# JiaoXianjun/multi-rtl-sdr-calibration

Hardware: AMD Instinct MI355X
Metric: IQ Msamples/s through FCCH+SCH calib (higher is better)
Workload: dtype f64; 1 GPU; cfg4 full chain gsm_sync_demod.m:107-124: 64 dongle streams (64/GPU) x 1020000 IQ samples (102 frames), fir1(46), FCCH+SCH+total_ppm_calculation, table on the host; streams_per_gpu=64, streams_total=64, output=table, collective=none, rows_checked_vs_oracle_per_rank=0

## Files before the change

### multi-rtl-sdr-calibration_amd/csrc/kernels_detect.h

```cpp
#pragma once
#include "state.h"
#include "kernels_frontend.h"

__device__ __forceinline__ constexpr int fft16_rev(int k) { return ((k & 1) << 3) | ((k & 2) << 1) | ((k & 4) >> 1) | ((k & 8) >> 3); }
__device__ __forceinline__ void fft16(cplx* x) {
    const double c1 = 0.92387953251128673848, s1 = 0.38268343236508978178;
    const double r2 = 0.70710678118654752440;
    const cplx w16[8] = {{1.0, 0.0}, {c1, -s1}, {r2, -r2}, {s1, -c1}, {0.0, -1.0}, {-s1, -c1}, {-r2, -r2}, {-c1, -s1}};
#pragma unroll
    for (int len = 16; len >= 2; len >>= 1) {
        const int half = len >> 1, step = 16 / len;
#pragma unroll
        for (int i = 0; i < 16; i += len) {
#pragma unroll
            for (int j = 0; j < half; ++j) {
                const cplx u = x[i + j], v = x[i + j + half];
                x[i + j] = make_double2(u.x + v.x, u.y + v.y);
                const cplx d = make_double2(u.x - v.x, u.y - v.y);
                const int t = j * step;
                if (t == 0) x[i + j + half] = d;
                else if (t == 4) x[i + j + half] = make_double2(d.y, -d.x);
                else x[i + j + half] = cmul(d, w16[t]);
            }
        }
// ... 1257 lines not shown
        qr = fma(u.x - v.x, t.y, qr); qi = fma(u.y - v.y, t.y, qi);
    }
    *Xa = make_double2(pr - qi, pi + qr);
    *Xb = make_double2(pr + qi, pi - qr);
}

__global__ void k_make_twiddles(cplx* tw, int n) {
    const int i = blockIdx.x * blockDim.x + threadIdx.x;
    if (i >= n) return;
    double sn, cs;
    sincospi(-2.0 * (double)i / (double)n, &sn, &cs);
    tw[i] = make_double2(cs, sn);
}

#define FFT_THREADS 512
#define FC_NB 8
template <int MODE>
__global__ void __launch_bounds__(FFT_THREADS) k_fft_burst(const StreamState* __restrict__ sts,
                                                           const cplx* __restrict__ win, long win_stream_stride,
                                                           long win_stride, int nfft,
                                                           const cplx* __restrict__ tw_g, PeakOut* __restrict__ peaks,
                                                           cplx* __restrict__ x0, int H) {
    extern __shared__ __attribute__((aligned(16))) unsigned char smem[];
    const int N2 = nfft / 37;
    const int ldb = N2 + 1;
    cplx* xs = (cplx*)smem;
    cplx* B = xs + nfft;
    cplx* w37 = B + 37 * ldb;
    cplx* wN2 = w37 + 40;
    __shared__ double red_p[FFT_THREADS / 64];
    __shared__ int red_t[FFT_THREADS / 64], red_k[FFT_THREADS / 64];
// ... 25 lines not shown
        const int ok = __shfl_down(key, off, 64);
        const int okk = __shfl_down(kk, off, 64);
        if (op > best || (op == best && ok < key)) { best = op; key = ok; kk = okk; }
    }
    const int wv = tid >> 6;
    if ((tid & 63) == 0) { red_p[wv] = best; red_t[wv] = key; red_k[wv] = kk; }
    __syncthreads();
    if (tid == 0) {
        for (int i = 1; i < FFT_THREADS / 64; ++i)
            if (red_p[i] > best || (red_p[i] == best && red_t[i] < key)) { best = red_p[i]; key = red_t[i]; kk = red_k[i]; }
        PeakOut o; o.p = best; o.tie = key; o.k = kk;
        peaks[(size_t)s * H + w] = o;
    }
}

#define FS_CHUNK 64
#define FS_ERR_SCALE_CHUNK 0.0001220703125

template <int NB = 19>
__device__ __forceinline__ cplx anchor_dft(const cplx* xw, int k, const cplx* __restrict__ tw_g, int nfft, int lane) {
    double ar = 0.0, ai = 0.0;
    const int stp = (int)(((unsigned)k * 64u) % (unsigned)nfft);
    int idx = (int)(((unsigned)k * (unsigned)lane) % (unsigned)nfft);
    for (int n0 = 0; n0 < nfft; n0 += NB * 64) {
        cplx t[NB];
        int id = idx;
#pragma unroll
        for (int u = 0; u < NB; ++u) {
            t[u] = tw_g[id];
            id += stp;
            if (id >= nfft) id -= nfft;
// ... 309 lines not shown
        if (res) *res = o2; else peak_store(&out[(size_t)s * H + w], o2);
    }
}

__device__ __forceinline__ float fc_group8_sum(float v) {
    int t;
    t = __builtin_amdgcn_update_dpp(0, __float_as_int(v), 0xB1, 0xF, 0xF, true);
    v += __int_as_float(t);
    t = __builtin_amdgcn_update_dpp(0, __float_as_int(v), 0x4E, 0xF, 0xF, true);
    v += __int_as_float(t);
    t = __builtin_amdgcn_update_dpp(0, __float_as_int(v), 0x141, 0xF, 0xF, true);
    v += __int_as_float(t);
    return v;
}

__host__ __device__ constexpr int fc_gcd64(int n) { int b = 64; while (n % b) b >>= 1; return b; }
__host__ __device__ constexpr int fc_threads(int nshift) {
    return ((nshift - 1) / FS_CHUNK * FC_NB + 63) / 64 * 64 < 256 ? 256 : ((nshift - 1) / FS_CHUNK * FC_NB + 63) / 64 * 64;
}
#define FC_XP(p) ((p) + ((p) >> 7))
struct FusedGather {
    const uint8_t* raw; long raw_stride;
    const double* coef;
    cplx* win_out;
    int ntaps, per;
    int sym47, pad;
};
__host__ inline size_t fc_stage_bytes(int per, int ntaps) {
    const int span8 = per + ntaps + 8;
    return (size_t)(span8 + span8 / 4 + 1) * sizeof(cplx) + (size_t)fir_taps_padded(ntaps) * sizeof(double);
}

struct FcCarve {
    int nstep, wlen, B, nA, nM, nchunk, ld1;
    size_t xs, reg1, reg2;
    size_t Sp, Et, tw1, tw2, sumS, Cs, sh_scan, sh_scan2;
    size_t total, launch, stage;
};
__host__ __device__ constexpr FcCarve fc_carve(int nshift, int nfft) {
    FcCarve c{};
    c.nstep = nshift - 1; c.wlen = c.nstep + nfft;
    c.B = fc_gcd64(nfft); c.nA = nfft / c.B; c.nM = c.wlen / c.B; c.nchunk = c.nstep / FS_CHUNK;
    c.ld1 = c.B + 2;
    const int xp = FC_XP(c.nstep + 2);
    const size_t r1 = (size_t)FC_NB * c.nM * sizeof(cplx), e1 = (size_t)(c.nstep + 2) * sizeof(double);
    const size_t r2 = (size_t)FC_NB * (c.B + 2 + nfft / c.B) * sizeof(cplx), e2 = (size_t)2 * (size_t)(xp + 1) * sizeof(float) + 16 * sizeof(double);
    c.xs = 0;
    c.reg1 = (size_t)FC_XP(c.wlen) * sizeof(cplx);
    c.reg2 = c.reg1 + (r1 > e1 ? r1 : e1);
    c.Sp = c.Et = c.reg1;
    c.tw1 = c.reg2;
    c.tw2 = c.tw1 + (size_t)(FC_NB * c.ld1) * sizeof(cplx);
    c.sumS = c.reg2;
    c.Cs = c.sumS + (size_t)xp * sizeof(float);
    c.sh_scan = c.Cs + (size_t)(xp + (xp & 1)) * sizeof(float);
    c.sh_scan2 = c.sh_scan + 8 * sizeof(double);
    c.total = c.reg2 + (r2 > e2 ? r2 : e2);
    c.launch = (c.total + 15) & ~(size_t)15;
    c.stage = c.launch - c.reg1 - 16;
    return c;
}
static_assert(fc_carve(1025, 1184).total == 53520, "reference geometry: with the 144 bytes of static LDS, 100 bytes under the 53 760-byte line (three workgroups per CU)");
template <typename T>
__device__ __forceinline__ T* fc_at(size_t off) {
    extern __shared__ __attribute__((aligned(16))) unsigned char smem[];
    return (T*)(smem + off);
}
struct FcThread { int tid, lane, wave, nthr, nwave; };
struct alignas(16) FcShared { double red_p[8]; int red_t[8], red_k[8]; int a, b, lo; };

#define FC_PRIO(P0, P1, P2) if (gridDim.x * gridDim.y <= 768u) { const unsigned rnd_ = (blockIdx.y * gridDim.x + blockIdx.x) >> 8; if (rnd_ == 0) __builtin_amdgcn_s_setprio(P0); else if (rnd_ == 1) __builtin_amdgcn_s_setprio(P1); else __builtin_amdgcn_s_setprio(P2); }
#define FC_PF 8
#ifdef GSMCAL_DEVTIMING
#define FC_ROLE_STAMP(wv, i)                                                                                          \
    do {                                                                                                              \
        if (DEV_STAMP_ON(KID_CERT, i) && g_stamps && th.wave == (wv) && th.lane == 0 && blockIdx.y * gridDim.x + blockIdx.x < DEV_STAMP_BLOCKS) \
            g_stamps[((size_t)KID_CERT * DEV_STAMP_BLOCKS + blockIdx.y * gridDim.x + blockIdx.x) * 16 + (i)] = wall_clock64();           \
// ... 186 lines not shown
    for (int a = 0; a < nA; ++a) {
        const cplx v = sb[a], t = tb[a * FC_NB];
        xr = fma(v.x, t.x, fma(-v.y, t.y, xr));
        xi = fma(v.x, t.y, fma(v.y, t.x, xi));
    }
}

__device__ __forceinline__ double fc_energy_term(const cplx& a1, const cplx& b1) {
    return (a1.x * a1.x + a1.y * a1.y) - (b1.x * b1.x + b1.y * b1.y);
}
__device__ __forceinline__ double fc_slack_term(const cplx& a1, const cplx& b1) {
    const double dr = a1.x - b1.x, di = a1.y - b1.y;
    return (double)(__fsqrt_rn((float)(dr * dr + di * di)) * 1.00000095367431640625f);
}

template <int OV>
__device__ __forceinline__ void fc_scan_role(const FcCarve& cv, const FcThread& th, int nfft, bool we) {
    const int lane = th.lane, nstep = cv.nstep;
    cplx* xs = fc_at<cplx>(cv.xs);
    double* Et = fc_at<double>(cv.Et);
    float* Cs = fc_at<float>(cv.Cs);
    const int per = OV > 0 ? 2 * OV : (nstep + 63) >> 6;
    const int i0 = lane * per < nstep ? lane * per : nstep, i1 = i0 + per < nstep ? i0 + per : nstep;
    auto term = [&](int q) -> double {
        const cplx a1 = xs[FC_XP(q + nfft)], b1 = xs[FC_XP(q)];
        if (we) return fc_energy_term(a1, b1);
        return fc_slack_term(a1, b1);
    };
    double run = 0.0;
    if (we) {
        for (int i = lane; i < nfft; i += 64) { const cplx v = xs[FC_XP(i)]; run += v.x * v.x + v.y * v.y; }
        for (int off = 32; off > 0; off >>= 1) run += __shfl_down(run, off, 64);
        run = __shfl(run, 0, 64);
    }
    double g[OV > 0 ? 2 * OV : 1];
    double loc = 0.0;
    if (OV > 0) {
#pragma unroll
        for (int u = 0; u < 2 * OV; ++u) { g[u] = term(i0 + u); loc += g[u]; }
    } else {
        for (int q = i0; q < i1; ++q) loc += term(q);
    }
    double inc = loc;
    for (int off = 1; off < 64; off <<= 1) {
        const double o = __shfl_up(inc, off, 64);
        if (lane >= off) inc += o;
    }
    const double exc = __shfl_up(inc, 1, 64);
    if (lane > 0) run += exc;
    if (OV > 0) {
#pragma unroll
        for (int u = 0; u < 2 * OV; ++u) {
            if (we) Et[i0 + u] = run; else Cs[FC_XP(i0 + u)] = (float)run;
            run += g[u];
        }
    } else {
        for (int q = i0; q < i1; ++q) {
            if (we) Et[q] = run; else Cs[FC_XP(q)] = (float)run;
            run += term(q);
        }
    }
    if (i1 == nstep && i0 < nstep) { if (we) Et[nstep] = run; else Cs[FC_XP(nstep)] = (float)run; }
}

__device__ __forceinline__ void fc_scan_block(const FcCarve& cv, const FcThread& th, int nfft, FcShared& sh) {
    const int tid = th.tid, lane = th.lane, wave = th.wave, nthr = th.nthr, nwave = th.nwave, nstep = cv.nstep;
    cplx* xs = fc_at<cplx>(cv.xs);
    double* Et = fc_at<double>(cv.Et);
    float* Cs = fc_at<float>(cv.Cs);
    double* sh_scan = fc_at<double>(cv.sh_scan);
    double* sh_scan2 = fc_at<double>(cv.sh_scan2);
    double e0 = 0.0;
    for (int i = tid; i < nfft; i += nthr) { const cplx v = xs[FC_XP(i)]; e0 += v.x * v.x + v.y * v.y; }
    for (int off = 32; off > 0; off >>= 1) e0 += __shfl_down(e0, off, 64);
    if (lane == 0) sh.red_p[wave] = e0;
    const int per = (nstep + nthr - 1) / nthr;
    const int i0 = tid * per < nstep ? tid * per : nstep, i1 = i0 + per < nstep ? i0 + per : nstep;
// ... 29 lines not shown
        const int ot = __shfl_down(bt, off, 64);
        const int ok = __shfl_down(bk, off, 64);
        if (op > best || (op == best && (ot < bt || (ot == bt && ok < bk)))) { best = op; bt = ot; bk = ok; }
    }
}
__device__ __forceinline__ void fc_block_best(const FcThread& th, FcShared& sh, double& best, int& bt, int& bk) {
    if (th.lane == 0) { sh.red_p[th.wave] = best; sh.red_t[th.wave] = bt; sh.red_k[th.wave] = bk; }
    __syncthreads();
    best = sh.red_p[0]; bt = sh.red_t[0]; bk = sh.red_k[0];
    for (int i = 1; i < th.nwave; ++i)
        if (sh.red_p[i] > best || (sh.red_p[i] == best && (sh.red_t[i] < bt || (sh.red_t[i] == bt && sh.red_k[i] < bk)))) {
            best = sh.red_p[i]; bt = sh.red_t[i]; bk = sh.red_k[i];
        }
}

__device__ __forceinline__ void fc_certificate(const FcCarve& cv, const FcThread& th, int nfft, FcShared& sh, double best, int bt) {
    const int tid = th.tid, lane = th.lane, wave = th.wave, nthr = th.nthr, nwave = th.nwave, nstep = cv.nstep;
    double* Et = fc_at<double>(cv.Et);
    float* sumS = fc_at<float>(cv.sumS);
    float* Cs = fc_at<float>(cv.Cs);
    double* sh_scan = fc_at<double>(cv.sh_scan);
    double* sh_scan2 = fc_at<double>(cv.sh_scan2);
    const double INF = __longlong_as_double(0x7ff0000000000000LL);
    const double sb = best > 0.0 ? sqrt(best) * (1.0 - 1e-9) : -1.0;
    const int per = (nstep + nthr) / nthr;
    const int u0 = tid * per < nstep + 1 ? tid * per : nstep + 1, u1 = u0 + per < nstep + 1 ? u0 + per : nstep + 1;
    double mf = INF, mb = INF;
    for (int t = u0; t < u1; ++t) {
        const double NE = (double)nfft * Et[t];
        const float ss = sumS[FC_XP(t)];
        const double R = NE - (double)ss + 4e-6 * NE;
        float sf = ss <= 3.0e38f ? __fsqrt_rn((float)(R > 0.0 ? R : 0.0)) * 1.000001f : __int_as_float(0x7f800000);
        if (!(sf >= 0.0f)) sf = __int_as_float(0x7f800000);
        sumS[FC_XP(t)] = sf;
        const double ct = (double)Cs[FC_XP(t)];
        mf = fmin(mf, (double)sf - ct);
        mb = fmin(mb, (double)sf + ct);
    }
    double pf = mf, pb = mb;
    for (int off = 1; off < 64; off <<= 1) {
        const double o = __shfl_up(pf, off, 64), ob = __shfl_down(pb, off, 64);
        if (lane >= off) pf = fmin(pf, o);
        if (lane + off < 64) pb = fmin(pb, ob);
    }
// ... 62 lines not shown
    FC_PRIO(0, 1, 2)
    if (fg.raw) {
        fc_window_raw<OV, NTAPS>(cv, th, fg, sts + s, (const unsigned short*)(fg.raw + (size_t)s * fg.raw_stride), sts[s].win_start[w],
                                 fg.win_out + (size_t)s * win_stream_stride + (size_t)w * win_stride);
        if (th.tid == 0) { sh.a = 0; sh.b = cv.nstep; }
        __syncthreads();
    } else {
        fc_window_load(cv, th, win + (size_t)s * win_stream_stride + (size_t)w * win_stride);
        if (th.tid == 0) { sh.a = 0; sh.b = cv.nstep; }
        __syncthreads();
    }
    DEV_STAMP(KID_CERT, blockIdx.y * gridDim.x + blockIdx.x, 1);
    FC_PRIO(2, 1, 0)
    const int lo = fc_choose_bins(cv, th, nfft, tw_g, sh);
    DEV_STAMP(KID_CERT, blockIdx.y * gridDim.x + blockIdx.x, 2);
    const int j = th.tid & (FC_NB - 1), c = th.tid / FC_NB;
    const bool act = c < cv.nchunk;
    const int k = ((lo + j) % nfft + nfft) % nfft;
    fc_twiddles(cv, th, nfft, lo, tw_g);
    __syncthreads();
    fc_level1(cv, th, j, c);
    __syncthreads();
    DEV_STAMP(KID_CERT, blockIdx.y * gridDim.x + blockIdx.x, 3);
    double xr = 0.0, xi = 0.0;
    if (act) fc_level2_anchor(cv, j, c, xr, xi);
    __syncthreads();
    DEV_STAMP(KID_CERT, blockIdx.y * gridDim.x + blockIdx.x, 4);
    FC_PRIO(0, 1, 2)
    const int nslide = (FC_NB * cv.nchunk + 63) >> 6;
    const bool split = th.nwave - nslide >= 2;
    if (split) {
        DEV_STAMP(KID_CERT, blockIdx.y * gridDim.x + blockIdx.x, 5);
        if (th.wave == nslide || th.wave == nslide + 1) {
            const bool we = th.wave == nslide;
            fc_scan_role<OV>(cv, th, nfft, we);
            FC_ROLE_STAMP(th.wave, we ? 12 : 13);
        }
    } else {
        fc_scan_block(cv, th, nfft, sh);
        DEV_STAMP(KID_CERT, blockIdx.y * gridDim.x + blockIdx.x, 5);
    }
    double best = -1.0;
    int bt = 0x7fffffff;
    if (act) {
        cplx* xs = fc_at<cplx>(cv.xs);
        float* sumS = fc_at<float>(cv.sumS);
        const cplx wk = tw_g[k];
        const double wr = wk.x, wi = -wk.y;
        const int t0 = c * FS_CHUNK;
        if (c == 0) {
            const double p = xr * xr + xi * xi;
// ... 17 lines not shown
                xi = ar * wi + ai * wr;
                const double p = xr * xr + xi * xi;
                if (p > best) { best = p; bt = t0 + q0 + u + 1; }
                ps[u] = fc_group8_sum((float)p);
            }
#pragma unroll
            for (int u = 0; u < FC_PF; ++u) sumS[FC_XP(t0 + q0 + u + 1)] = ps[u];
        }
    }
    FC_ROLE_STAMP(0, 14);
    int bk = k;
    fc_wave_best(best, bt, bk);
    __syncthreads();
    DEV_STAMP(KID_CERT, blockIdx.y * gridDim.x + blockIdx.x, 6);
    fc_block_best(th, sh, best, bt, bk);
    fc_certificate(cv, th, nfft, sh, best, bt);
    __syncthreads();
#ifdef GSMCAL_AB_LAZY_WIN
    if (fg.raw && OV > 0 && NTAPS == 47 && fg.sym47 != 0 && (sh.a != 0 || sh.b < cv.nstep)) {
        cplx* wout = fg.win_out + (size_t)s * win_stream_stride + (size_t)w * win_stride;
        const cplx* xs = fc_at<cplx>(cv.xs);
        for (int i = th.tid; i < cv.wlen; i += th.nthr) wout[i] = xs[FC_XP(i)];
    }
#endif
    if (th.tid == 0) fc_emit(cv, sh, best, bt, bk, s, H, w, cert, items, n_items);
    DEV_STAMP(KID_CERT, blockIdx.y * gridDim.x + blockIdx.x, 7);
}

__global__ void __launch_bounds__(256) k_fine_search(const StreamState* __restrict__ sts,
                                                     const cplx* __restrict__ win, long win_stream_stride,
                                                     long win_stride, int nshift, int nfft,
// ... 95 lines not shown
```

Before: 568,100 Msample/s.

## Rework split-role prefix scans with DPP wave scans and interleaved chunk mapping

The energy and slack prefix scans in the split-role path now take strided shifts (lane + 64u) and use a DPP-based f64 inclusive wave scan, replacing the per-lane contiguous ranges and shfl_up scan. The initial-window energy term moves out of the energy wave into the slack wave and is added as e0 in the certificate step, which shortens the energy wave's critical path. Sliding-sum chunks are remapped across waves (fc_slide_chunk) so each slide wave covers interleaved chunks. Layout constants move into a shared header. A Python LDS bank-conflict model is added for profiling.

After: 574,500 Msample/s (median of 6 runs). +1.1%, better.

```diff
diff --git a/multi-rtl-sdr-calibration_amd/csrc/fc_layout.h b/multi-rtl-sdr-calibration_amd/csrc/fc_layout.h
--- /dev/null
+++ b/multi-rtl-sdr-calibration_amd/csrc/fc_layout.h
@@ -0,0 +1,57 @@
+#pragma once
+#include <stddef.h>
+
+#if defined(__HIPCC__)
+#define FC_HD __host__ __device__
+#else
+#define FC_HD
+#endif
+
+#define FC_NB 8
+#define FS_CHUNK 64
+#define FC_CPLX_BYTES 16
+
+FC_HD constexpr int fc_gcd64(int n) { int b = 64; while (n % b) b >>= 1; return b; }
+FC_HD constexpr int fc_threads(int nshift) {
+    return ((nshift - 1) / FS_CHUNK * FC_NB + 63) / 64 * 64 < 256 ? 256 : ((nshift - 1) / FS_CHUNK * FC_NB + 63) / 64 * 64;
+}
+#define FC_XP(p) ((p) + ((p) >> 7))
+
+struct FcCarve {
+    int nstep, wlen, B, nA, nM, nchunk, ld1;
+    size_t xs, reg1, reg2;
+    size_t Sp, Et, tw1, tw2, sumS, Cs, sh_scan, sh_scan2;
+    size_t total, launch, stage;
+};
+FC_HD constexpr FcCarve fc_carve(int nshift, int nfft) {
+    FcCarve c{};
+    c.nstep = nshift - 1; c.wlen = c.nstep + nfft;
+    c.B = fc_gcd64(nfft); c.nA = nfft / c.B; c.nM = c.wlen / c.B; c.nchunk = c.nstep / FS_CHUNK;
+    c.ld1 = c.B + 2;
+    const int xp = FC_XP(c.nstep + 2);
+    const size_t r1 = (size_t)FC_NB * c.nM * FC_CPLX_BYTES, e1 = (size_t)(c.nstep + 2) * sizeof(double);
+    const size_t r2 = (size_t)FC_NB * (c.B + 2 + nfft / c.B) * FC_CPLX_BYTES, e2 = (size_t)2 * (size_t)(xp + 1) * sizeof(float) + 16 * sizeof(double);
+    c.xs = 0;
+    c.reg1 = (size_t)FC_XP(c.wlen) * FC_CPLX_BYTES;
+    c.reg2 = c.reg1 + (r1 > e1 ? r1 : e1);
+    c.Sp = c.Et = c.reg1;
+    c.tw1 = c.reg2;
+    c.tw2 = c.tw1 + (size_t)(FC_NB * c.ld1) * FC_CPLX_BYTES;
+    c.sumS = c.reg2;
+    c.Cs = c.sumS + (size_t)xp * sizeof(float);
+    c.sh_scan = c.Cs + (size_t)(xp + (xp & 1)) * sizeof(float);
+    c.sh_scan2 = c.sh_scan + 8 * sizeof(double);
+    c.total = c.reg2 + (r2 > e2 ? r2 : e2);
+    c.launch = (c.total + 15) & ~(size_t)15;
+    c.stage = c.launch - c.reg1 - 16;
+    return c;
+}
+static_assert(fc_carve(1025, 1184).total == 53520, "reference geometry: with the 144 bytes of static LDS, 100 bytes under the 53 760-byte line (three workgroups per CU)");
+
+FC_HD constexpr int fc_nslide(int nchunk) { return (FC_NB * nchunk + 63) >> 6; }
+#define FC_NO_CHUNK (1 << 20)
+FC_HD constexpr int fc_slide_chunk(int tid, int nslide) {
+    return (tid >> 6) < nslide ? nslide * ((tid & 63) / FC_NB) + (tid >> 6) : FC_NO_CHUNK;
+}
+FC_HD constexpr int fc_scan_rounds(int nstep) { return (nstep + 63) >> 6; }
+FC_HD constexpr int fc_scan_shift(int lane, int u) { return lane + 64 * u; }
diff --git a/multi-rtl-sdr-calibration_amd/csrc/kernels_detect.h b/multi-rtl-sdr-calibration_amd/csrc/kernels_detect.h
--- a/multi-rtl-sdr-calibration_amd/csrc/kernels_detect.h
+++ b/multi-rtl-sdr-calibration_amd/csrc/kernels_detect.h
@@ -1,6 +1,7 @@
 #pragma once
 #include "state.h"
 #include "kernels_frontend.h"
+#include "fc_layout.h"
 
 __device__ __forceinline__ constexpr int fft16_rev(int k) { return ((k & 1) << 3) | ((k & 2) << 1) | ((k & 4) >> 1) | ((k & 8) >> 3); }
 __device__ __forceinline__ void fft16(cplx* x) {
@@ -1295,7 +1296,6 @@
 }
 
 #define FFT_THREADS 512
-#define FC_NB 8
 template <int MODE>
 __global__ void __launch_bounds__(FFT_THREADS) k_fft_burst(const StreamState* __restrict__ sts,
                                                            const cplx* __restrict__ win, long win_stream_stride,
@@ -1351,7 +1351,6 @@
     }
 }
 
-#define FS_CHUNK 64
 #define FS_ERR_SCALE_CHUNK 0.0001220703125
 
 template <int NB = 19>
@@ -1691,11 +1690,6 @@
     return v;
 }
 
-__host__ __device__ constexpr int fc_gcd64(int n) { int b = 64; while (n % b) b >>= 1; return b; }
-__host__ __device__ constexpr int fc_threads(int nshift) {
-    return ((nshift - 1) / FS_CHUNK * FC_NB + 63) / 64 * 64 < 256 ? 256 : ((nshift - 1) / FS_CHUNK * FC_NB + 63) / 64 * 64;
-}
-#define FC_XP(p) ((p) + ((p) >> 7))
 struct FusedGather {
     const uint8_t* raw; long raw_stride;
     const double* coef;
@@ -1708,36 +1702,7 @@
     return (size_t)(span8 + span8 / 4 + 1) * sizeof(cplx) + (size_t)fir_taps_padded(ntaps) * sizeof(double);
 }
 
-struct FcCarve {
-    int nstep, wlen, B, nA, nM, nchunk, ld1;
-    size_t xs, reg1, reg2;
-    size_t Sp, Et, tw1, tw2, sumS, Cs, sh_scan, sh_scan2;
-    size_t total, launch, stage;
-};
-__host__ __device__ constexpr FcCarve fc_carve(int nshift, int nfft) {
-    FcCarve c{};
-    c.nstep = nshift - 1; c.wlen = c.nstep + nfft;
-    c.B = fc_gcd64(nfft); c.nA = nfft / c.B; c.nM = c.wlen / c.B; c.nchunk = c.nstep / FS_CHUNK;
-    c.ld1 = c.B + 2;
-    const int xp = FC_XP(c.nstep + 2);
-    const size_t r1 = (size_t)FC_NB * c.nM * sizeof(cplx), e1 = (size_t)(c.nstep + 2) * sizeof(double);
-    const size_t r2 = (size_t)FC_NB * (c.B + 2 + nfft / c.B) * sizeof(cplx), e2 = (size_t)2 * (size_t)(xp + 1) * sizeof(float) + 16 * sizeof(double);
-    c.xs = 0;
-    c.reg1 = (size_t)FC_XP(c.wlen) * sizeof(cplx);
-    c.reg2 = c.reg1 + (r1 > e1 ? r1 : e1);
-    c.Sp = c.Et = c.reg1;
-    c.tw1 = c.reg2;
-    c.tw2 = c.tw1 + (size_t)(FC_NB * c.ld1) * sizeof(cplx);
-    c.sumS = c.reg2;
-    c.Cs = c.sumS + (size_t)xp * sizeof(float);
-    c.sh_scan = c.Cs + (size_t)(xp + (xp & 1)) * sizeof(float);
-    c.sh_scan2 = c.sh_scan + 8 * sizeof(double);
-    c.total = c.reg2 + (r2 > e2 ? r2 : e2);
-    c.launch = (c.total + 15) & ~(size_t)15;
-    c.stage = c.launch - c.reg1 - 16;
-    return c;
-}
-static_assert(fc_carve(1025, 1184).total == 53520, "reference geometry: with the 144 bytes of static LDS, 100 bytes under the 53 760-byte line (three workgroups per CU)");
+static_assert(sizeof(cplx) == FC_CPLX_BYTES, "fc_carve() counts samples of 16 bytes");
 template <typename T>
 __device__ __forceinline__ T* fc_at(size_t off) {
     extern __shared__ __attribute__((aligned(16))) unsigned char smem[];
@@ -1954,53 +1919,59 @@
     return (double)(__fsqrt_rn((float)(dr * dr + di * di)) * 1.00000095367431640625f);
 }
 
-template <int OV>
-__device__ __forceinline__ void fc_scan_role(const FcCarve& cv, const FcThread& th, int nfft, bool we) {
+template <int CTRL, int ROW_MASK>
+__device__ __forceinline__ double fc_dpp_f64(double v) {
+    const int lo = __builtin_amdgcn_update_dpp(0, __double2loint(v), CTRL, ROW_MASK, 0xF, ROW_MASK == 0xF);
+    const int hi = __builtin_amdgcn_update_dpp(0, __double2hiint(v), CTRL, ROW_MASK, 0xF, ROW_MASK == 0xF);
+    return __hiloint2double(hi, lo);
+}
+__device__ __forceinline__ double fc_wave_scan(double v) {
+    v += fc_dpp_f64<0x111, 0xF>(v);
+    v += fc_dpp_f64<0x112, 0xF>(v);
+    v += fc_dpp_f64<0x114, 0xF>(v);
+    v += fc_dpp_f64<0x118, 0xF>(v);
+    v += fc_dpp_f64<0x142, 0xA>(v);
+    v += fc_dpp_f64<0x143, 0xC>(v);
+    return v;
+}
+
+template <int OV, bool WE>
+__device__ __forceinline__ void fc_scan_role(const FcCarve& cv, const FcThread& th, int nfft, double* e0) {
     const int lane = th.lane, nstep = cv.nstep;
     cplx* xs = fc_at<cplx>(cv.xs);
     double* Et = fc_at<double>(cv.Et);
     float* Cs = fc_at<float>(cv.Cs);
-    const int per = OV > 0 ? 2 * OV : (nstep + 63) >> 6;
-    const int i0 = lane * per < nstep ? lane * per : nstep, i1 = i0 + per < nstep ? i0 + per : nstep;
-    auto term = [&](int q) -> double {
+    double run = 0.0;
+    auto term = [&](int u) -> double {
+        const int q = fc_scan_shift(lane, u);
+        if (OV == 0 && q >= nstep) return 0.0;
         const cplx a1 = xs[FC_XP(q + nfft)], b1 = xs[FC_XP(q)];
-        if (we) return fc_energy_term(a1, b1);
-        return fc_slack_term(a1, b1);
+        return WE ? fc_energy_term(a1, b1) : fc_slack_term(a1, b1);
     };
-    double run = 0.0;
-    if (we) {
-        for (int i = lane; i < nfft; i += 64) { const cplx v = xs[FC_XP(i)]; run += v.x * v.x + v.y * v.y; }
-        for (int off = 32; off > 0; off >>= 1) run += __shfl_down(run, off, 64);
-        run = __shfl(run, 0, 64);
-    }
-    double g[OV > 0 ? 2 * OV : 1];
-    double loc = 0.0;
+    auto scan = [&](int u, double g) {
+        const int q = fc_scan_shift(lane, u);
+        const double inc = fc_wave_scan(g);
+        const double at = run + fc_dpp_f64<0x138, 0xF>(inc);
+        if (OV > 0 || q < nstep) { if (WE) Et[q] = at; else Cs[FC_XP(q)] = (float)at; }
+        run += __hiloint2double(__builtin_amdgcn_readlane(__double2hiint(inc), 63), __builtin_amdgcn_readlane(__double2loint(inc), 63));
+    };
     if (OV > 0) {
-#pragma unroll
-        for (int u = 0; u < 2 * OV; ++u) { g[u] = term(i0 + u); loc += g[u]; }
+        double g[OV > 0 ? 2 * OV : 1];
+#pragma unroll
+        for (int u = 0; u < 2 * OV; ++u) g[u] = term(u);
+#pragma unroll
+        for (int u = 0; u < 2 * OV; ++u) scan(u, g[u]);
     } else {
-        for (int q = i0; q < i1; ++q) loc += term(q);
-    }
-    double inc = loc;
-    for (int off = 1; off < 64; off <<= 1) {
-        const double o = __shfl_up(inc, off, 64);
-        if (lane >= off) inc += o;
-    }
-    const double exc = __shfl_up(inc, 1, 64);
-    if (lane > 0) run += exc;
-    if (OV > 0) {
-#pragma unroll
-        for (int u = 0; u < 2 * OV; ++u) {
-            if (we) Et[i0 + u] = run; else Cs[FC_XP(i0 + u)] = (float)run;
-            run += g[u];
-        }
-    } else {
-        for (int q = i0; q < i1; ++q) {
-            if (we) Et[q] = run; else Cs[FC_XP(q)] = (float)run;
-            run += term(q);
-        }
-    }
-    if (i1 == nstep && i0 < nstep) { if (we) Et[nstep] = run; else Cs[FC_XP(nstep)] = (float)run; }
+        const int rounds = fc_scan_rounds(nstep);
+        for (int u = 0; u < rounds; ++u) scan(u, term(u));
+    }
+    if (lane == 0) { if (WE) Et[nstep] = run; else Cs[FC_XP(nstep)] = (float)run; }
+    if (!WE) {
+        double e = 0.0;
+        for (int i = lane; i < nfft; i += 64) { const cplx v = xs[FC_XP(i)]; e += v.x * v.x + v.y * v.y; }
+        for (int off = 32; off > 0; off >>= 1) e += __shfl_down(e, off, 64);
+        if (lane == 0) *e0 = e;
+    }
 }
 
 __device__ __forceinline__ void fc_scan_block(const FcCarve& cv, const FcThread& th, int nfft, FcShared& sh) {
@@ -2060,7 +2031,7 @@
         }
 }
 
-__device__ __forceinline__ void fc_certificate(const FcCarve& cv, const FcThread& th, int nfft, FcShared& sh, double best, int bt) {
+__device__ __forceinline__ void fc_certificate(const FcCarve& cv, const FcThread& th, int nfft, FcShared& sh, double best, int bt, double e0) {
     const int tid = th.tid, lane = th.lane, wave = th.wave, nthr = th.nthr, nwave = th.nwave, nstep = cv.nstep;
     double* Et = fc_at<double>(cv.Et);
     float* sumS = fc_at<float>(cv.sumS);
@@ -2073,7 +2044,7 @@
     const int u0 = tid * per < nstep + 1 ? tid * per : nstep + 1, u1 = u0 + per < nstep + 1 ? u0 + per : nstep + 1;
     double mf = INF, mb = INF;
     for (int t = u0; t < u1; ++t) {
-        const double NE = (double)nfft * Et[t];
+        const double NE = (double)nfft * (Et[t] + e0);
         const float ss = sumS[FC_XP(t)];
         const double R = NE - (double)ss + 4e-6 * NE;
         float sf = ss <= 3.0e38f ? __fsqrt_rn((float)(R > 0.0 ? R : 0.0)) * 1.000001f : __int_as_float(0x7f800000);
@@ -2166,12 +2137,13 @@
     FC_PRIO(2, 1, 0)
     const int lo = fc_choose_bins(cv, th, nfft, tw_g, sh);
     DEV_STAMP(KID_CERT, blockIdx.y * gridDim.x + blockIdx.x, 2);
-    const int j = th.tid & (FC_NB - 1), c = th.tid / FC_NB;
+    const int nslide = fc_nslide(cv.nchunk);
+    const int j = th.tid & (FC_NB - 1), c1 = th.tid / FC_NB, c = fc_slide_chunk(th.tid, nslide);
     const bool act = c < cv.nchunk;
     const int k = ((lo + j) % nfft + nfft) % nfft;
     fc_twiddles(cv, th, nfft, lo, tw_g);
     __syncthreads();
-    fc_level1(cv, th, j, c);
+    fc_level1(cv, th, j, c1);
     __syncthreads();
     DEV_STAMP(KID_CERT, blockIdx.y * gridDim.x + blockIdx.x, 3);
     double xr = 0.0, xi = 0.0;
@@ -2179,14 +2151,16 @@
     __syncthreads();
     DEV_STAMP(KID_CERT, blockIdx.y * gridDim.x + blockIdx.x, 4);
     FC_PRIO(0, 1, 2)
-    const int nslide = (FC_NB * cv.nchunk + 63) >> 6;
     const bool split = th.nwave - nslide >= 2;
     if (split) {
         DEV_STAMP(KID_CERT, blockIdx.y * gridDim.x + blockIdx.x, 5);
-        if (th.wave == nslide || th.wave == nslide + 1) {
-            const bool we = th.wave == nslide;
-            fc_scan_role<OV>(cv, th, nfft, we);
-            FC_ROLE_STAMP(th.wave, we ? 12 : 13);
+        const int role = __builtin_amdgcn_readfirstlane(th.wave) - nslide;
+        if (role == 0) {
+            fc_scan_role<OV, true>(cv, th, nfft, nullptr);
+            FC_ROLE_STAMP(th.wave, 12);
+        } else if (role == 1) {
+            fc_scan_role<OV, false>(cv, th, nfft, fc_at<double>(cv.sh_scan2) + 7);
+            FC_ROLE_STAMP(th.wave, 13);
         }
     } else {
         fc_scan_block(cv, th, nfft, sh);
@@ -2234,7 +2208,8 @@
     __syncthreads();
     DEV_STAMP(KID_CERT, blockIdx.y * gridDim.x + blockIdx.x, 6);
     fc_block_best(th, sh, best, bt, bk);
-    fc_certificate(cv, th, nfft, sh, best, bt);
+    const double e0 = split ? fc_at<double>(cv.sh_scan2)[7] : 0.0;
+    fc_certificate(cv, th, nfft, sh, best, bt, e0);
     __syncthreads();
 #ifdef GSMCAL_AB_LAZY_WIN
     if (fg.raw && OV > 0 && NTAPS == 47 && fg.sym47 != 0 && (sh.a != 0 || sh.b < cv.nstep)) {
diff --git a/profiles/fc_bank_model.py b/profiles/fc_bank_model.py
--- /dev/null
+++ b/profiles/fc_bank_model.py
@@ -0,0 +1,184 @@
+#!/usr/bin/env python3
+import sys
+from collections import defaultdict
+
+NSHIFT, NFFT, NTHR, NB, PER, NTAPS = 1025, 1184, 256, 8, 736, 47
+NSTEP = NSHIFT - 1
+WLEN = NSTEP + NFFT
+B, NA, NM, LD1, NCHUNK = 32, 37, 69, 34, 16
+STATIC = 144
+
+
+def XP(p):
+    return p + (p >> 7)
+
+
+def xs_pad(p):
+    return p + (p >> 2)
+
+
+XS = 0
+REG1 = XP(WLEN) * 16
+REG2 = REG1 + NB * NM * 16
+SUMS = REG2
+CS = SUMS + XP(NSTEP + 2) * 4
+TW1 = REG2
+TW2 = TW1 + NB * LD1 * 16
+
+G128 = [0, 0, 0, 0, 1, 1, 1, 1, 1, 1, 1, 1, 0, 0, 0, 0, 1, 1, 1, 1, 0, 0, 0, 0, 0, 0, 0, 0, 1, 1, 1, 1]
+KINDS = {
+    "r128": (64, 4, lambda l: 2 * (l >> 5) + G128[l & 31]),
+    "r64": (64, 2, lambda l: l >> 5),
+    "r32": (32, 1, lambda l: l >> 5),
+    "w128": (32, 4, lambda l: l >> 3),
+    "w64": (32, 2, lambda l: l >> 4),
+    "w32": (32, 1, lambda l: l >> 5),
+}
+
+
+def extra(kind, addr):
+    nb, dw, grp = KINDS[kind]
+    on = defaultdict(lambda: defaultdict(set))
+    for l, a in addr.items():
+        a += STATIC
+        for d in range(dw):
+            on[grp(l)][(a // 4 + d) % nb].add(a)
+    ways = [max(len(s) for s in banks.values()) for banks in on.values()]
+    return sum(w - 1 for w in ways), max(ways) if ways else 0
+
+
+class Table:
+    def __init__(self):
+        self.rows = defaultdict(lambda: [0, 0, 0])
+
+    def add(self, site, kind, fn, lanes_of_wave=None):
+        for w in range(NTHR // 64):
+            addr = {}
+            for l in range(64):
+                a = fn(64 * w + l)
+                if a is not None:
+                    addr[l] = a
+            if addr:
+                e, wy = extra(kind, addr)
+                r = self.rows[site]
+                r[0] += 1; r[1] += e; r[2] = max(r[2], wy)
+
+
+def model(new, off=3):
+    t = Table()
+    for o0 in range(0, WLEN, PER):
+        cnt = min(PER, WLEN - o0)
+        span = cnt + NTAPS - 1
+        for off in (off,):
+            r = (-off) & 3
+            for u in range(8):
+                def f(tid, u=u):
+                    ib = 8 * tid - off
+                    if ib < 0 or ib + 8 > span + 8:
+                        return None
+                    return REG1 + (xs_pad(ib) + u + ((r + u) >> 2)) * 16 if ib + 8 <= span else (REG1 + xs_pad(ib + u) * 16 if ib + u < span + 8 else None)
+                t.add("raw_chunk_to_lds: xq stores (w128, lanes 10 slots apart)", "w128", f)
+        for s in range(50):
+            t.add("fir4_sym47: xq reads (r128, lanes 5 slots apart)", "r128",
+                  lambda tid, s=s: REG1 + (xs_pad(4 * tid) + s + (s >> 2)) * 16 if 4 * tid < cnt else None)
+        for k in range(4):
+            t.add("fc_window_raw: xs stores (w128, lanes 4 slots apart)", "w128",
+                  lambda tid, k=k: XS + XP(o0 + 4 * tid + k) * 16 if 4 * tid + k < cnt else None)
+    n0 = NSTEP // 2
+    for i in range(8):
+        t.add("fc_choose_bins: decimating read (r128, lanes 8 slots apart)", "r128",
+              lambda tid, i=i: XS + XP(n0 + 8 * tid + i) * 16 if tid < 148 else None)
+    t.add("fc_choose_bins: yd / t148 stores (w128)", "w128", lambda tid: REG1 + tid * 16 if tid < 148 else None)
+    t.add("fc_choose_bins: yd / t148 stores (w128)", "w128", lambda tid: REG1 + (148 + tid) * 16 if tid < 148 else None)
+    PW = REG1 + 296 * 16
+    A = PW + 148 * 8
+    for n1 in range(37):
+        t.add("fc_choose_bins: 37-point stage (r128: yd broadcast, t148 scattered)", "r128",
+              lambda tid, n1=n1: REG1 + (4 * n1 + tid // 37) * 16 if tid < 148 else None)
+        t.add("fc_choose_bins: 37-point stage (r128: yd broadcast, t148 scattered)", "r128",
+              lambda tid, n1=n1: REG1 + (148 + (4 * (tid % 37) * n1) % 148) * 16 if tid < 148 else None)
+    t.add("fc_choose_bins: A / pw stores", "w128", lambda tid: A + tid * 16 if tid < 148 else None)
+    for n2 in range(4):
+        t.add("fc_choose_bins: 4-point stage (r128)", "r128", lambda tid, n2=n2: A + (n2 * 37 + tid % 37) * 16 if tid < 148 else None)
+        t.add("fc_choose_bins: 4-point stage (r128)", "r128", lambda tid, n2=n2: REG1 + (148 + (tid * n2) % 148) * 16 if tid < 148 else None)
+    t.add("fc_choose_bins: A / pw stores", "w64", lambda tid: PW + tid * 8 if tid < 148 else None)
+    for r in range(3):
+        t.add("fc_choose_bins: pw reads of wave 0 (r64)", "r64", lambda tid, r=r: PW + (tid + 64 * r) * 8 if tid < 64 and tid + 64 * r < 148 else None)
+    t.add("fc_twiddles: tw1 / tw2 stores (w128)", "w128", lambda tid: TW1 + ((tid // B) * LD1 + tid % B) * 16)
+    for r in range(2):
+        t.add("fc_twiddles: tw1 / tw2 stores (w128)", "w128",
+              lambda tid, r=r: TW2 + (tid + 256 * r) * 16 if tid + 256 * r < NB * NA else None)
+    for r in range(3):
+        for i in range(B):
+            def m_of(tid, r=r):
+                m = tid // NB + 32 * r
+                return m if m < NM else None
+            t.add("fc_level1: xs reads (r128, start rotated by group)", "r128",
+                  lambda tid, i=i: None if m_of(tid) is None else XS + (XP(B * m_of(tid)) + ((tid // NB + i) & (B - 1))) * 16)
+            t.add("fc_level1: tw1 reads (r128, plane stride 34)", "r128",
+                  lambda tid, i=i: None if m_of(tid) is None else TW1 + ((tid % NB) * LD1 + ((tid // NB + i) & (B - 1))) * 16)
+        t.add("fc_level1: Sp stores (w128, j rows 69 apart)", "w128",
+              lambda tid: None if m_of(tid) is None else REG1 + ((tid % NB) * NM + m_of(tid)) * 16)
+
+    def chunk(tid):
+        if new:
+            return 2 * ((tid & 63) >> 3) + (tid >> 6) if (tid >> 6) < 2 else None
+        return tid // NB if tid // NB < NCHUNK else None
+    for a in range(NA):
+        t.add("fc_level2_anchor: Sp reads (r128: j rows 69 apart, chunks 2 apart)", "r128",
+              lambda tid, a=a: None if chunk(tid) is None else REG1 + ((tid % NB) * NM + 2 * chunk(tid) + a) * 16)
+        t.add("fc_level2_anchor: tw2 reads (r128, 8 consecutive)", "r128",
+              lambda tid, a=a: None if chunk(tid) is None else TW2 + (a * NB + tid % NB) * 16)
+    for r in range(19):
+        t.add("fc_scan_role: E(0) reads (r128, consecutive)", "r128",
+              lambda tid, r=r: XS + XP(tid - 128 + 64 * r) * 16 if 128 <= tid < 192 and tid - 128 + 64 * r < NFFT else None)
+    for u in range(16):
+        q = (lambda tid, u=u: (tid & 63) + 64 * u) if new else (lambda tid, u=u: 16 * (tid & 63) + u)
+        t.add("fc_scan_role: x[q + nfft], x[q] reads (r128)", "r128", lambda tid: XS + XP(q(tid) + NFFT) * 16 if tid >= 128 else None)
+        t.add("fc_scan_role: x[q + nfft], x[q] reads (r128)", "r128", lambda tid: XS + XP(q(tid)) * 16 if tid >= 128 else None)
+        t.add("fc_scan_role: Et stores (w64)", "w64", lambda tid: REG1 + q(tid) * 8 if 128 <= tid < 192 else None)
+        t.add("fc_scan_role: Cs stores (w32)", "w32", lambda tid: CS + XP(q(tid)) * 4 if tid >= 192 else None)
+    for qq in range(64):
+        t.add("slides: x[t + nfft], x[t] reads (r128, 8 lanes per address)", "r128",
+              lambda tid: None if chunk(tid) is None else XS + XP(64 * chunk(tid) + NFFT + qq) * 16)
+        t.add("slides: x[t + nfft], x[t] reads (r128, 8 lanes per address)", "r128",
+              lambda tid: None if chunk(tid) is None else XS + XP(64 * chunk(tid) + qq) * 16)
+        t.add("slides: sumS stores (w32, 8 lanes per address)", "w32",
+              lambda tid: None if chunk(tid) is None else SUMS + XP(64 * chunk(tid) + qq + 1) * 4)
+    for k in range(5):
+        tt = lambda tid, k=k: 5 * tid + k if 5 * tid + k <= NSTEP else None
+        t.add("fc_certificate: Et reads (r64, lanes 40 bytes apart)", "r64", lambda tid: None if tt(tid) is None else REG1 + tt(tid) * 8)
+        for rep in range(3):
+            t.add("fc_certificate: sumS / Cs reads (r32, lanes 20 bytes apart)", "r32", lambda tid: None if tt(tid) is None else SUMS + XP(tt(tid)) * 4)
+            t.add("fc_certificate: sumS / Cs reads (r32, lanes 20 bytes apart)", "r32", lambda tid: None if tt(tid) is None else CS + XP(tt(tid)) * 4)
+        t.add("fc_certificate: s(t) stores (w32)", "w32", lambda tid: None if tt(tid) is None else SUMS + XP(tt(tid)) * 4)
+    return t
+
+
+def main():
+    argv = sys.argv[1:]
+    windows, off = 626, None
+    if "--windows" in argv:
+        i = argv.index("--windows"); windows = int(argv[i + 1]); del argv[i:i + 2]
+    if "--off" in argv:
+        i = argv.index("--off"); off = int(argv[i + 1]); del argv[i:i + 2]
+    which = argv or ["parent", "new"]
+    tabs = {w: model(w == "new", 3 if off is None else off) for w in which}
+    sites = list(next(iter(tabs.values())).rows)
+    print("| site | wave instr | " + " | ".join(f"extra cycles ({w}) | ways ({w})" for w in which) + " |")
+    print("|---|---|" + "---|---|" * len(which))
+    for s in sites:
+        print(f"| {s} | {tabs[which[0]].rows[s][0]} | " + " | ".join(f"{tabs[w].rows[s][1]} | {tabs[w].rows[s][2]}" for w in which) + " |")
+    for w in which:
+        tot = sum(r[1] for r in tabs[w].rows.values())
+        ins = sum(r[0] for r in tabs[w].rows.values())
+        print(f"{w}: {ins} modelled wave instructions, {tot} extra cycles per workgroup; x {windows} working workgroups = "
+              f"{tot * windows / 1e6:.2f} M per launch (x 752 launched = {tot * 752 / 1e6:.2f} M)")
+    if off is None:
+        for w in which:
+            tots = [sum(r[1] for r in model(w == "new", o).rows.values()) for o in range(8)]
+            print(f"{w}: extra cycles per workgroup by staging offset 0..7: {tots} (spread {100.0 * (max(tots) - min(tots)) / min(tots):.1f} %)")
+
+
+if __name__ == "__main__":
+    main()
diff --git a/profiles/tail_bank_model.py b/profiles/tail_bank_model.py
--- /dev/null
+++ b/profiles/tail_bank_model.py
@@ -0,0 +1,263 @@
+#!/usr/bin/env python3
+import sys
+from collections import defaultdict
+
+from fc_bank_model import extra
+
+NT = 512
+
+
+class Table:
+    def __init__(self):
+        self.rows = defaultdict(lambda: [0, 0, 0])
+
+    def add(self, site, kind, fn, nthr=NT):
+        for w in range(nthr // 64):
+            addr = {l: fn(64 * w + l) for l in range(64)}
+            addr = {l: a for l, a in addr.items() if a is not None}
+            if addr:
+                e, wy = extra(kind, addr)
+                r = self.rows[site]
+                r[0] += 1; r[1] += e; r[2] = max(r[2], wy)
+
+    def show(self, title, windows, measured_inst, measured_conf):
+        print(f"### {title}")
+        print("| site | wave instr | ways | extra / workgroup |")
+        print("|---|---|---|---|")
+        for s, r in self.rows.items():
+            print(f"| {s} | {r[0]} | {r[2]} | {r[1]} |")
+        ins = sum(r[0] for r in self.rows.values()); tot = sum(r[1] for r in self.rows.values())
+        print(f"| **total** | {ins} | | **{tot}** |")
+        print(f"{tot} x {windows} working workgroups = {tot * windows / 1e6:.3f} M per launch, measured {measured_conf / 1e6:.3f} M "
+              f"({100.0 * (tot * windows - measured_conf) / measured_conf:+.0f} %); modelled LDS instructions {ins * windows / 1e6:.3f} M "
+              f"of {measured_inst / 1e6:.3f} M measured\n")
+
+
+def xs_pad(p):
+    return p + (p >> 2)
+
+
+def gather_carve(length, level, ntaps, compact):
+    bufn = length + 40
+    span_max = length + 8 + ntaps + 24
+    xs_n = span_max + 16 if compact else span_max + span_max // 4 + 16
+    r1 = max(bufn, xs_n)
+    off_region1 = bufn * 16
+    off_coef = off_region1 + r1 * 16
+    off_raw = off_coef + ((ntaps + 3) & ~3) * 8
+    total = (off_raw + ((span_max + 7) & ~7) * 2 + 15) & ~15
+    off_rot = off_raw
+    rot_end = off_rot + (1 + 72 + 32) * 16
+    if level >= 2 and rot_end > total:
+        total = (rot_end + 15) & ~15
+    return dict(bufn=bufn, r1=off_region1, coef=off_coef, rot=off_rot, total=total)
+
+
+def window_sch(off=3):
+    t = Table()
+    L, NTAPS, NSH, LT = 600, 47, 89, 512
+    gc = gather_carve(L, 2, NTAPS, False)
+    BUF0, BUF1, CS, T = 0, gc["r1"], gc["coef"], gc["rot"]
+    cnt0 = L + 1
+    span = cnt0 + NTAPS - 1
+    nchunk = (off + span + 15) >> 3
+    for u in range(8):
+        t.add("sch_gather_fast: staged input stores (w128, lanes 10 slots apart)", "w128",
+              lambda tid, u=u: BUF1 + xs_pad(8 * tid - off + u) * 16 if tid < nchunk and 0 <= 8 * tid - off + u < span + 8 else None)
+    nwc = (nchunk + 63) >> 6
+    t.add("sch_gather_fast: rotator table and tap stores", "w128",
+          lambda tid: T + (tid - 64 * nwc) * 16 if 0 <= tid - 64 * nwc < 52 else None)
+    t.add("sch_gather_fast: rotator table and tap stores", "w64",
+          lambda tid: CS + (tid - 64 * nwc - 64) * 8 if 0 <= tid - 64 * nwc - 64 < 48 else None)
+    act = lambda tid: 4 * tid < cnt0
+    for k in range(4):
+        t.add("fir4_lds: sample reads (r128, lanes 5 slots apart)", "r128", lambda tid, k=k: BUF1 + (xs_pad(4 * tid) + k) * 16 if act(tid) else None)
+    for tr in range(12):
+        for h in range(2):
+            t.add("fir4_lds: tap reads (r128, one address)", "r128", lambda tid, tr=tr, h=h: CS + (4 * tr + 2 * h) * 8 if act(tid) else None)
+        for k in range(4):
+            t.add("fir4_lds: sample reads (r128, lanes 5 slots apart)", "r128",
+                  lambda tid, tr=tr, k=k: BUF1 + (xs_pad(4 * tid + 4 * tr + 4) + k) * 16 if act(tid) else None)
+    for k in range(4):
+        t.add("sch_gather_fast: level-0 stores (w128, lanes 4 slots apart)", "w128",
+              lambda tid, k=k: BUF0 + (4 * tid + k) * 16 if 4 * tid + k < cnt0 else None)
+    for r in range(2):
+        i_of = lambda tid, r=r: tid + 512 * r if tid + 512 * r < L else None
+        for d in range(2):
+            t.add("sch_gather_fast: interpolation reads (r128, consecutive)", "r128",
+                  lambda tid, d=d: None if i_of(tid) is None else BUF0 + (i_of(tid) + d) * 16)
+        t.add("sch_gather_fast: rotator reads S, A[i >> 5], B[i & 31] (r128)", "r128", lambda tid: None if i_of(tid) is None else T)
+        t.add("sch_gather_fast: rotator reads S, A[i >> 5], B[i & 31] (r128)", "r128",
+              lambda tid: None if i_of(tid) is None else T + (1 + (i_of(tid) >> 5)) * 16)
+        t.add("sch_gather_fast: rotator reads S, A[i >> 5], B[i & 31] (r128)", "r128",
+              lambda tid: None if i_of(tid) is None else T + (1 + 72 + (i_of(tid) & 31)) * 16)
+        t.add("sch_gather_fast: window stores (w128, consecutive)", "w128", lambda tid: None if i_of(tid) is None else BUF1 + i_of(tid) * 16)
+    R, Q, M = 4, 16, 39
+    NG = (NSH + R - 1) // R
+    PADL, NTC, WL = R * NG, R * NG + Q * M, NSH - 1 + LT
+    TC = gc["total"]
+    CV = TC + (LT + NSH * 4) * 16
+    for r in range(2):
+        t.add("sch_corr_rows: padded tap copy and zero stores (w128, consecutive)", "w128",
+              lambda tid, r=r: TC + (tid + 512 * r) * 16 if tid + 512 * r < NTC else None)
+    t.add("sch_corr_rows: padded tap copy and zero stores (w128, consecutive)", "w128", lambda tid: BUF1 + (WL + tid) * 16 if WL + tid < Q * M else None)
+    on = lambda tid: tid < NG * Q
+    for s in (-1, -2, -3):
+        t.add("sch_corr_rows: tap reads tp[s] (r128: stretches 39 slots apart, offset groups 4 apart)", "r128",
+              lambda tid, s=s: TC + (PADL + (tid & 15) * M - R * (tid >> 4) + s) * 16 if on(tid) else None)
+    for s in range(M):
+        t.add("sch_corr_rows: sample reads xp[s] (r128: stretches 39 slots apart, 4 rows per address)", "r128",
+              lambda tid, s=s: BUF1 + ((tid & 15) * M + s) * 16 if on(tid) else None)
+        t.add("sch_corr_rows: tap reads tp[s] (r128: stretches 39 slots apart, offset groups 4 apart)", "r128",
+              lambda tid, s=s: TC + (PADL + (tid & 15) * M - R * (tid >> 4) + s) * 16 if on(tid) else None)
+    t.add("sch_corr_rows: power stores, argmax reads (w64 / r64)", "w64",
+          lambda tid: CV + (R * (tid >> 4) + (tid & 15)) * 8 if on(tid) and (tid & 15) < R and R * (tid >> 4) + (tid & 15) < NSH else None)
+    for r in range(2):
+        t.add("sch_corr_rows: power stores, argmax reads (w64 / r64)", "r64", lambda tid, r=r: CV + (tid + 64 * r) * 8 if tid < 64 and tid + 64 * r < NSH else None)
+    return t
+
+
+def burst_tone(gate, kbin, jm):
+    t = Table()
+    N, N2, LDB = 1184, 32, 33
+    gc = gather_carve(N, 1 if gate else 3, 47, True)
+    BUF0, BUF1 = 0, gc["r1"]
+    T = gc["rot"]
+    W37 = gc["total"]
+    WN2 = W37 + 40 * 16
+    P = WN2 + N2 * 16
+    rounds = lambda n: range((n + NT - 1) // NT)
+    idx = lambda tid, r, n: tid + NT * r if tid + NT * r < n else None
+    for r in rounds(N):
+        t.add("burst_gather_fast: twiddle table and window stores (w128, consecutive)", "w128", lambda tid, r=r: None if idx(tid, r, N) is None else BUF1 + idx(tid, r, N) * 16)
+        t.add("burst_gather_fast: twiddle table and window stores (w128, consecutive)", "w128", lambda tid, r=r: None if idx(tid, r, N) is None else BUF0 + idx(tid, r, N) * 16)
+    if not gate:
+        for r in rounds(N):
+            t.add("burst_gather_fast: level-1 stores (w128, consecutive)", "w128", lambda tid, r=r: None if idx(tid, r, N) is None else BUF1 + idx(tid, r, N) * 16)
+            for d in range(2):
+                t.add("burst_gather_fast: level-1 reads for level 3 (r128, consecutive)", "r128",
+                      lambda tid, r=r, d=d: None if idx(tid, r, N) is None else BUF1 + (idx(tid, r, N) + d) * 16)
+                t.add("burst_gather_fast: rotator reads S, A[i >> 5], B[i & 31] (r128)", "r128", lambda tid, r=r: None if idx(tid, r, N) is None else T)
+                t.add("burst_gather_fast: rotator reads S, A[i >> 5], B[i & 31] (r128)", "r128",
+                      lambda tid, r=r, d=d: None if idx(tid, r, N) is None else T + (1 + ((idx(tid, r, N) + d) >> 5)) * 16)
+                t.add("burst_gather_fast: rotator reads S, A[i >> 5], B[i & 31] (r128)", "r128",
+                      lambda tid, r=r, d=d: None if idx(tid, r, N) is None else T + (1 + 72 + ((idx(tid, r, N) + d) & 31)) * 16)
+    for r in rounds(N):
+        t.add("energy: xs reads (r128, consecutive)", "r128", lambda tid, r=r: None if idx(tid, r, N) is None else BUF0 + idx(tid, r, N) * 16)
+    for r in range((N + 63) // 64):
+        t.add("candidate DFTs: xs reads (r128, consecutive)", "r128",
+              lambda tid, r=r: BUF0 + ((tid & 63) + 64 * r) * 16 if tid < 448 and (tid & 63) + 64 * r < N else None)
+        t.add("candidate DFTs: twiddle reads twl[(k n) mod nfft] (r128, lanes k slots apart)", "r128",
+              lambda tid, r=r: BUF1 + (((kbin - 3 + (tid >> 6)) % N * ((tid & 63) + 64 * r)) % N) * 16 if tid < 448 and (tid & 63) + 64 * r < N else None)
+    for r in rounds(N - 1):
+        for d in range(2):
+            t.add("phase estimate: xs[n], xs[n + 1] reads (r128, consecutive)", "r128",
+                  lambda tid, r=r, d=d: None if idx(tid, r, N - 1) is None else BUF0 + (idx(tid, r, N - 1) + d) * 16)
+            t.add("phase estimate: twiddle reads twl[(n j) mod nfft] (r128, lanes j slots apart)", "r128",
+                  lambda tid, r=r, d=d: None if idx(tid, r, N - 1) is None else BUF1 + (((idx(tid, r, N - 1) + d) * jm) % N) * 16)
+    if gate:
+        PW, BASE = P, P + 16 * 16
+        for r in range(2):
+            o_of = lambda tid, r=r: tid + NT * r if tid + NT * r < 19 * N2 else None
+            def ia(tid):
+                o = o_of(tid)
+                return None if o is None else (o - 18 * N2 if o >= 18 * N2 else N2 * (1 + o // N2) + o % N2)
+            def ib(tid):
+                o = o_of(tid)
+                return None if o is None or o >= 18 * N2 else N2 * (36 - o // N2) + o % N2
+            for f in (ia, ib):
+                t.add("gate, pass A: xs reads and stores (r128 / w128, runs of 32)", "r128", lambda tid, f=f: None if f(tid) is None else BUF0 + f(tid) * 16)
+                t.add("gate, pass A: xs reads and stores (r128 / w128, runs of 32)", "w128", lambda tid, f=f: None if f(tid) is None else BUF0 + f(tid) * 16)
+                t.add("gate, pass A: twiddle reads twl[(n j) mod nfft] (r128, lanes j slots apart)", "r128",
+                      lambda tid, f=f: None if f(tid) is None else BUF1 + ((f(tid) * jm) % N) * 16)
+                t.add("gate, pass A: base[n >> 4], pw[n & 15] reads (r128)", "r128", lambda tid, f=f: None if f(tid) is None else BASE + (f(tid) >> 4) * 16)
+                t.add("gate, pass A: base[n >> 4], pw[n & 15] reads (r128)", "r128", lambda tid, f=f: None if f(tid) is None else PW + (f(tid) & 15) * 16)
+        BB = BUF1
+        for r in range(2):
+            o_of = lambda tid, r=r: tid + NT * r if tid + NT * r < 19 * N2 else None
+            t.add("gate, pass B: xs and w37 reads (r128, runs of 32 / one address per run)", "r128", lambda tid: None if o_of(tid) is None else BUF0 + (o_of(tid) % N2) * 16)
+            for n1 in range(1, 19):
+                t.add("gate, pass B: xs and w37 reads (r128, runs of 32 / one address per run)", "r128",
+                      lambda tid, n1=n1: None if o_of(tid) is None else BUF0 + (N2 * n1 + o_of(tid) % N2) * 16)
+                t.add("gate, pass B: xs and w37 reads (r128, runs of 32 / one address per run)", "r128",
+                      lambda tid, n1=n1: None if o_of(tid) is None else BUF0 + (N2 * (37 - n1) + o_of(tid) % N2) * 16)
+                t.add("gate, pass B: xs and w37 reads (r128, runs of 32 / one address per run)", "r128",
+                      lambda tid, n1=n1: None if o_of(tid) is None else W37 + ((n1 * (o_of(tid) // N2)) % 37) * 16)
+            t.add("gate, pass B: B stores (w128, rows 33 apart)", "w128", lambda tid: None if o_of(tid) is None else BB + ((o_of(tid) // N2) * LDB + o_of(tid) % N2) * 16)
+            t.add("gate, pass B: B stores (w128, rows 33 apart)", "w128",
+                  lambda tid: None if o_of(tid) is None or o_of(tid) < N2 else BB + ((37 - o_of(tid) // N2) * LDB + o_of(tid) % N2) * 16)
+        kk = lambda tid: None if tid >= 176 else (tid if tid < 88 else N - 176 + tid)
+        for n2 in range(N2):
+            t.add("gate, step 2: B row reads (r128, rows 33 apart)", "r128", lambda tid, n2=n2: None if kk(tid) is None else BB + ((kk(tid) % 37) * LDB + n2) * 16)
+            t.add("gate, step 2: wN2[(n2 k2) mod 32] reads (r128, a few addresses per wave)", "r128",
+                  lambda tid, n2=n2: None if kk(tid) is None else WN2 + ((n2 * (kk(tid) // 37)) % N2) * 16)
+        t.add("gate: band power stores and reads (w64 / r64, consecutive)", "w64", lambda tid: None if tid >= 176 else P + tid * 8)
+        for r in range(3):
+            t.add("gate: band power stores and reads (w64 / r64, consecutive)", "r64", lambda tid, r=r: P + (3 + tid + 64 * r) * 8 if tid < 64 and 3 + tid + 64 * r < 174 else None)
+    return t
+
+
+def fine_chunk():
+    t = Table()
+    FK, N, N2, LDB = 640, 1184, 32, 33
+    XS = 0
+    BB = (N + 64) * 16
+    W37 = BB + 37 * LDB * 16
+    WN2 = W37 + 40 * 16
+    D = WN2 + N2 * 16
+    idx = lambda tid, r, n: tid + FK * r if tid + FK * r < n else None
+    for r in range(2):
+        t.add("window copy and error-bound reads (w128 / r128, consecutive)", "w128", lambda tid, r=r: None if idx(tid, r, N + 64) is None else XS + idx(tid, r, N + 64) * 16, FK)
+        t.add("window copy and error-bound reads (w128 / r128, consecutive)", "r128", lambda tid, r=r: None if idx(tid, r, N) is None else XS + idx(tid, r, N) * 16, FK)
+    t.add("steps d[t]: reads and store (r128 / w64, consecutive)", "r128", lambda tid: XS + (tid + N) * 16 if tid < 64 else None, FK)
+    t.add("steps d[t]: reads and store (r128 / w64, consecutive)", "r128", lambda tid: XS + tid * 16 if tid < 64 else None, FK)
+    t.add("steps d[t]: reads and store (r128 / w64, consecutive)", "w64", lambda tid: D + tid * 8 if tid < 64 else None, FK)
+    ia = lambda tid: N2 * (1 + tid // N2) + tid % N2 if tid < 18 * N2 else None
+    ib = lambda tid: N2 * (36 - tid // N2) + tid % N2 if tid < 18 * N2 else None
+    for f in (ia, ib):
+        t.add("fft37_step1_sym, pass A: xs reads and stores (runs of 32)", "r128", lambda tid, f=f: None if f(tid) is None else XS + f(tid) * 16, FK)
+        t.add("fft37_step1_sym, pass A: xs reads and stores (runs of 32)", "w128", lambda tid, f=f: None if f(tid) is None else XS + f(tid) * 16, FK)
+    on = lambda tid: tid < 19 * N2
+    t.add("fft37_step1_sym, pass B: xs and w37 reads (runs of 32 / one address per run)", "r128", lambda tid: XS + (tid % N2) * 16 if on(tid) else None, FK)
+    for n1 in range(1, 19):
+        t.add("fft37_step1_sym, pass B: xs and w37 reads (runs of 32 / one address per run)", "r128", lambda tid, n1=n1: XS + (N2 * n1 + tid % N2) * 16 if on(tid) else None, FK)
+        t.add("fft37_step1_sym, pass B: xs and w37 reads (runs of 32 / one address per run)", "r128", lambda tid, n1=n1: XS + (N2 * (37 - n1) + tid % N2) * 16 if on(tid) else None, FK)
+        t.add("fft37_step1_sym, pass B: xs and w37 reads (runs of 32 / one address per run)", "r128", lambda tid, n1=n1: W37 + ((n1 * (tid // N2)) % 37) * 16 if on(tid) else None, FK)
+    t.add("fft37_step1_sym, pass B: B stores (w128, rows 33 apart)", "w128", lambda tid: BB + ((tid // N2) * LDB + tid % N2) * 16 if on(tid) else None, FK)
+    t.add("fft37_step1_sym, pass B: B stores (w128, rows 33 apart)", "w128", lambda tid: BB + ((37 - tid // N2) * LDB + tid % N2) * 16 if on(tid) and tid >= N2 else None, FK)
+    row = lambda tid: BB + (tid % 37) * LDB * 16
+    for n2 in range(N2):
+        t.add("fft37_step2_pair, j = 0: B row reads (r128, rows 33 apart)", "r128", lambda tid, n2=n2: row(tid) + n2 * 16 if tid < 37 else None, FK)
+    gen = lambda tid: 37 <= tid < N // 2
+    for n2 in (0, 16):
+        t.add("fft37_step2_pair: B row reads (r128, rows 33 apart, wrapping at row 37)", "r128", lambda tid, n2=n2: row(tid) + n2 * 16 if gen(tid) else None, FK)
+    for n2 in range(1, 16):
+        t.add("fft37_step2_pair: B row reads (r128, rows 33 apart, wrapping at row 37)", "r128", lambda tid, n2=n2: row(tid) + n2 * 16 if gen(tid) else None, FK)
+        t.add("fft37_step2_pair: B row reads (r128, rows 33 apart, wrapping at row 37)", "r128", lambda tid, n2=n2: row(tid) + (N2 - n2) * 16 if gen(tid) else None, FK)
+        t.add("fft37_step2_pair: wN2[(n2 j) mod 32] reads (r128, two or three addresses per wave)", "r128",
+              lambda tid, n2=n2: WN2 + ((n2 * (tid // 37)) % N2) * 16 if gen(tid) else None, FK)
+    for tt in range(64):
+        t.add("sweep: d[t] reads (r64, one address)", "r64", lambda tid, tt=tt: D + tt * 8 if tid < N // 2 else None, FK)
+    return t
+
+
+def main():
+    argv = sys.argv[1:]
+    opt = lambda name, d: int(argv[argv.index(name) + 1]) if name in argv else d
+    kbin = opt("--bin", 37)
+    window_sch().show("k_window_sch<8, 512, 47> (per launch: 576 207 LDS instructions, 773 950 conflict cycles)", opt("--sch-windows", 580), 576207, 773950)
+    burst_tone(1, kbin, kbin).show(f"k_burst_tone<1, 8, 47> with the tone at bin {kbin} (per launch: 872 712 LDS instructions, 1 102 056 conflict cycles)",
+                                   opt("--burst-windows", 626), 872712, 1102056)
+    tots = {k: sum(r[1] for r in burst_tone(1, k, k).rows.values()) for k in range(17, 58)}
+    print("k_burst_tone<1>: extra cycles per workgroup by the tone's bin 17..57:", list(tots.values()))
+    for lo, hi in ((27, 47), (17, 57)):
+        m = sum(tots[k] for k in range(lo, hi + 1)) / (hi - lo + 1)
+        print(f"  mean over bins {lo}..{hi}: {m:.0f} per workgroup, x 626 = {m * 626 / 1e6:.3f} M per launch (measured 1.102 M, {100.0 * (m * 626 - 1102056) / 1102056:+.0f} %)")
+    print()
+    fine_chunk().show("k_fine_chunk, per open (window, chunk) item (per launch: 278 511 LDS instructions, 139 717 conflict cycles, 214 items)",
+                      opt("--chunk-items", 214), 278511, 139717)
+    burst_tone(0, 37, 37).show("k_burst_tone<0, 8, 47>: carrier corrected, tone at bin 37 (per launch: 452 519 LDS instructions, 559 185 conflict cycles)", opt("--burst0-windows", 560), 452519, 559185)
+
+
+if __name__ == "__main__":
+    main()
```
